# PolusAI/nyxus

Measured on AMD Instinct MI355X. Metric: ROIs/sec (*ALL_GLCM*+*ALL_INTENSITY*, 1024^2 tiles), higher is better.
Workload: dtype f64; 1 GPU; *ALL_GLCM*+*ALL_INTENSITY*, coarse_gray_depth=8, 4 angles, d=1, 1000 synthetic 1024x1024 tiles/GPU x 196 ROIs/tile (disk r=30, 2821 px, bbox 61x61), intensities U[1,4095]; reduce stage on pre-assembled ROI clouds resident in HBM; n_columns=185

## Files before the change

nyxus_amd/csrc/intensity_close.h:

```cpp
#pragma once
#include <hip/hip_runtime.h>
#include "device_math.h"
#include "glcm_rows.h"

namespace nyxhip {

struct RowColumns {
    double* o;
    __device__ __forceinline__ double& operator()(int c) const { return o[c]; }
};

template <class OUT, class SLIDE>
__device__ __forceinline__ void close_sums(const OUT& O, double dn, uint32_t vmin, uint32_t vmax, double tot, double totsq, double mean,
                                           bool have_slide, const SLIDE& slide_range, bool blank)
{
    O(I_MIN) = (double)vmin;
    O(I_MAX) = (double)vmax;
    O(I_RANGE) = (double)vmax - (double)vmin;
    if (have_slide)
        O(I_COVERED_IMAGE_INTENSITY_RANGE) = (double)(vmax - vmin) / slide_range();
    O(I_MEAN) = mean;
    O(I_ENERGY) = totsq;
    O(I_ROOT_MEAN_SQUARED) = sqrt(totsq / dn);
    O(I_INTEGRATED_INTENSITY) = tot;
// ... 50 lines not shown
        const double M2 = acc[1], M3 = acc[2], M4 = acc[3];
        if (M2 != 0.0) {
            const double kurt = n > 4 ? (dn * M4) / (M2 * M2) : 0.0;
            O(I_SKEWNESS) = n > 3 ? (sqrt(dn) * M3) / (M2 * sqrt(M2)) : 0.0;
            O(I_KURTOSIS) = kurt;
            O(I_EXCESS_KURTOSIS) = n > 4 ? kurt - 3 : 0.0;
        }
        const double sd2 = sd * sd, d5 = dn * (sd2 * sd2 * sd), d6 = dn * (sd2 * sd2 * sd2);
        O(I_HYPERSKEWNESS) = d5 == 0. ? 0. : acc[4] / d5;
        O(I_HYPERFLATNESS) = d6 == 0. ? 0. : acc[5] / d6;
    }
}

template <class OUT>
__device__ __forceinline__ void close_robust_mad(const OUT& O, double sadk, uint32_t m2x, uint32_t cle, uint32_t K, double Sx, uint32_t vmin, double dn)
{
    const double dK = (double)K;
    const double sadt = 2.0 * sadk + ((m2x & 1u) ? 2.0 * (double)cle - dn : 0.0);
    O(I_ROBUST_MEAN) = K ? (Sx + dK * (double)vmin) / dK : 0.0;
    O(I_MEDIAN_ABSOLUTE_DEVIATION) = fdiv(sadt * 0.5, dn);
}
template <class OUT>
__device__ __forceinline__ void close_robust_rmad(const OUT& O, double adin, bool fast32, uint32_t K, double Sx, uint32_t lox, uint32_t hix,
                                                  uint32_t n_below, uint32_t n_above)
{
    const double dK = (double)K;
    if (fast32) {
        const double klo = (double)K * (double)lox, khi = (double)K * (double)hix;
        adin -= (double)n_below * fabs(klo - Sx) + (double)n_above * fabs(khi - Sx);
    }
    O(I_ROBUST_MEAN_ABSOLUTE_DEVIATION) = K ? fdiv(fdiv(adin, dK), dK) : 0.0;
}

template <class OUT>
__device__ __forceinline__ void close_quartiles(const OUT& O, double p25, double p75)
{
    O(I_QCOD) = (p75 - p25) / (p75 + p25);
    O(I_INTERQUARTILE_RANGE) = p75 - p25;
}

}
```

nyxus_amd/csrc/roi_features.hip:

```cpp
#include <hip/hip_runtime.h>
#include <type_traits>
#include <algorithm>
#include <cstdlib>
#include <cstdio>
#include "device_math.h"
#include "roi_kernel.h"
#include "launch_util.h"
#include "glcm_rows.h"
#include "glcm_w64.h"
#include "intensity_close.h"
#include "sort_lds.h"
#include "../../include/nyxhip.h"

namespace nyxhip {


enum { S_MEAN = 0, S_P10, S_P90, S_MEDIAN, S_MODE, S_NG };


template <int NW> __device__ __forceinline__ double xw_chain(const double* s_red, int k)
{
    return NW == 1 ? s_red[k] : ((s_red[k] + s_red[8 + k]) + s_red[16 + k]) + s_red[24 + k];
}
template <int NW> __device__ __forceinline__ double xw_pairs(const double* s_red, int k)
{
    return NW == 1 ? s_red[k] : (s_red[k] + s_red[8 + k]) + (s_red[16 + k] + s_red[24 + k]);
}

template <int N, bool GS, int NW = 4>
__device__ __forceinline__ void block_sum(double (&v)[N], double* s_red, int tid)
{
    const int lane = tid & 63, wave = __builtin_amdgcn_readfirstlane(tid >> 6);
    if (N > 4) {
        double t[8];
#pragma unroll
        for (int k = 0; k < 8; k++) t[k] = k < N ? v[k] : 0.0;
        const double tot = wave_transpose_sum8(t, lane);
        if ((lane & 7) == 0 && (lane >> 3) < N)
            s_red[wave * 8 + (lane >> 3)] = tot;
    } else if (N > 2) {
        double t[4];
#pragma unroll
        for (int k = 0; k < 4; k++) t[k] = k < N ? v[k] : 0.0;
        const double tot = wave_transpose_sum4(t);
        if ((lane & 15) == 0 && (lane >> 4) < N)
            s_red[wave * 8 + (lane >> 4)] = tot;
    } else {
#pragma unroll
        for (int k = 0; k < N; k++)
            v[k] = wave_sum(v[k]);
// ... 599 lines not shown
        lds_cu16_t* pc = (lds_cu16_t*)(uintptr_t)(Pd + cj);
        unsigned long long rem = __ballot(act && rc != 0u);
        while (rem) {
            const int r = (int)__builtin_ctzll(rem);
            rem &= rem - 1ull;
            const uint32_t cnt = pc[r * pitch];
            if (cnt >= 7u) { const double p = (double)cnt * inv_sum_p; ent += p * (double)fast_log2f(p + 0.000000001); }
        }
    }
    if constexpr (ROLE == 1) {
        blk_sync<false>();
        blk_sync<false>();
        hxy1c = T2[lane];
        hxy2 = f[lane];
        wav_sync<false>();
    }
    G16_EXIT(5, (uint32_t)(pcol + prow + pxmy + pxpy[0] + pxpy[1] + ent + hxy1c + hxy2) + asm_i + cmax);
    glcm_w64_tail<NG>(Ng, lane, rc, cc, dc, pxpy_c, csum, sum_p, inv_sum_p, pcol, prow, pxmy, pxpy, ent, hxy1c, hxy2, asm_i, cmax, f);
}

#ifdef NYX_STAMP
#define STAMP(i)                                                                          \
    do {                                                                                  \
        unsigned long long t__ = __builtin_readcyclecounter();                            \
        if (tid == 0 && A.stamps) atomicAdd(&A.stamps[i], t__ - t_prev__);                \
        t_prev__ = __builtin_readcyclecounter();                                          \
    } while (0)
#elif defined(NYX_EXIT_AT)
#define STAMP(i) do { if ((i) == NYX_EXIT_AT) return; } while (0)
#else
#define STAMP(i) do { } while (0)
#endif

typedef __attribute__((address_space(3))) uint8_t lds_u8_t;

typedef const __attribute__((address_space(4))) RoiArgs KArgs;
__device__ __forceinline__ KArgs* late_kernarg()
{
    KArgs* p = (KArgs*)__builtin_amdgcn_kernarg_segment_ptr();
    asm volatile("" : "+s"(p));
    return p;
}
template <bool LATE>
struct KView {
    const RoiArgs& a;
    KArgs* p;
    __device__ __forceinline__ explicit KView(const RoiArgs& a_) : a(a_), p(LATE ? late_kernarg() : nullptr) {}
    __device__ __forceinline__ auto operator->() const
    {
        if constexpr (LATE) return p;
        else return &a;
    }
};
template <bool GS, bool C16, bool SPLIT, bool D8, int FAM = 0, int TIER = 4, bool G16 = false, int WIN = 2, int NW = 4, bool DEFER_P = false>
__device__ __forceinline__ void roi_features_body(const RoiArgs& A, const uint64_t slot)
{
    static_assert((NW == 4 && NW == kMaxAngles) || (NW == 8 && G16 && FAM == 4), "one workgroup of four waves per ROI (and a wave per GLCM angle)");
    constexpr int BS = NW * 64;
    extern __shared__ __attribute__((aligned(16))) unsigned char lds_raw[];
    unsigned char* const lds = GS ? A.sp.scratch + (size_t)blockIdx.x * A.sp.stride : lds_raw;
    const int tid = (int)threadIdx.x, lane = tid & 63, wave = __builtin_amdgcn_readfirstlane(tid >> 6);
    uint64_t roi;
    if (!roi_of_slot(A.sp, slot, A.n_roi, roi))
        return;

    auto reg = [&](uint32_t o) -> unsigned char* { return (GS && o < A.L.gs_lds_bytes) ? lds_raw + o : lds + o; };
// ... 23 lines not shown
    const bool do_glcm = FAM == 1 || FAM == 3 || FAM == 4 || (FAM == 0 && (A.mask & NYXHIP_FAM_GLCM) != 0);
    double* const out_row = A.out + roi * A.ld;
#ifdef NYX_STAMP
    unsigned long long t_prev__ = __builtin_readcyclecounter();
#endif

    const uint32_t range = vmax - vmin;
    const bool use_count = C16 ? do_int : (do_int && A.L.count_cap != 0 && range < A.L.count_cap);
    if (C16 && do_int && range >= A.L.count_cap) {
        if (tid == 0) atomicCAS(A.status, 0, NYXHIP_ERR_ROI_TOO_LARGE);
        return;
    }
    uint32_t* s_cnt = (uint32_t*)reg(A.L.cnt);
    uint32_t P2 = 1;
    while (P2 < n)
        P2 <<= 1;
    const bool radix = !C16 && A.L.radix != 0;
    const bool k16 = radix && A.L.radix_k16 != 0;
    if (n == 0 || (do_int && ((use_count || radix) ? n : P2) > A.L.sort_cap) || (do_glcm && area > A.L.dense_cap)) {
        if (SPLIT && A.glcm_ng && tid == 0)
            A.glcm_ng[roi] = 0;
        if (n != 0 && A.sp.defer_large)
            return;
        if (tid == 0 && n != 0)
            atomicCAS(A.status, 0, NYXHIP_ERR_ROI_TOO_LARGE);
        for (int c = tid; c < A.n_cols; c += BS)
            out_row[c] = __longlong_as_double(0x7ff8000000000000LL);
        return;
    }

    const int greyInfo = A.ibsi ? 0 : A.grey_depth;
    if (FAST) __builtin_assume(greyInfo > 0 && greyInfo <= 16);
    if (G16) __builtin_assume(greyInfo > 16 && greyInfo <= 64);
    const double mslope = greyInfo > 0 ? (double)greyInfo / ((double)vmax - 0.) : 0.0;

    for (int c = tid; c < A.n_cols; c += BS)
        out_row[c] = 0.0;
    if (do_glcm) {
        uint32_t* d32 = (uint32_t*)s_dense;
        for (uint32_t i = tid; i < (D8 ? (area + 64 + 3) / 4 : (area + 1) / 2); i += BS)
            d32[i] = 0;
        if (greyInfo < 0)
            for (uint32_t i = tid; i <= A.L.lvl_cap; i += BS)
                s_lvlmap[i] = 0;
    }
    if (do_int) {
        if (use_count) {
            uint4* c4 = (uint4*)s_cnt;
            const uint32_t n16 = C16 ? (range + 8) / 8 : (range + 4) / 4;
            for (uint32_t i = tid; i < n16; i += BS)
                c4[i] = make_uint4(0, 0, 0, 0);
        } else if (!radix) {
            for (uint32_t i = n + tid; i < P2; i += BS)
                s_val[i] = 0xFFFFFFFFu;
        }
    }
    if (tid < 16)
        s_stat[tid] = 0.0;
    grp_sync<GS, NW>();

    STAMP(0);
    unsigned long long sum = 0, sumsq = 0;
    uint32_t lvl_max = 0;
    constexpr int kU = 4;
    const bool small_v = vmax < (1u << 24);
    const __amdgpu_buffer_rsrc_t rs_v = __builtin_amdgcn_make_buffer_rsrc((void*)(A.inten + off), 0, (int)(n * 4u), 0x00020000);
    const __amdgpu_buffer_rsrc_t rs_x = __builtin_amdgcn_make_buffer_rsrc((void*)(A.x + off), 0, (int)(n * 2u), 0x00020000);
    const __amdgpu_buffer_rsrc_t rs_y = __builtin_amdgcn_make_buffer_rsrc((void*)(A.y + off), 0, (int)(n * 2u), 0x00020000);
    auto trip = [&](auto full_c, auto nz_c, auto tiny_c, uint32_t base) {
        constexpr bool FULL = decltype(full_c)::value, NZ = decltype(nz_c)::value, TINY = decltype(tiny_c)::value;
        uint32_t v[kU], px[kU], py[kU];
#pragma unroll
        for (int u = 0; u < kU; u++) {
            const uint32_t i = base + u * BS + tid;
            v[u] = __builtin_amdgcn_raw_buffer_load_b32(rs_v, (int)(i * 4u), 0, 0);
            px[u] = do_glcm ? (uint32_t)(uint16_t)__builtin_amdgcn_raw_buffer_load_b16(rs_x, (int)(i * 2u), 0, 0) : 0u;
            py[u] = do_glcm ? (uint32_t)(uint16_t)__builtin_amdgcn_raw_buffer_load_b16(rs_y, (int)(i * 2u), 0, 0) : 0u;
        }
        uint32_t s32 = 0, q32 = 0;
        const uint32_t i0 = base + tid;
        uint16_t* const val16 = (uint16_t*)s_val + i0;
#pragma unroll
        for (int u = 0; u < kU; u++) {
            if (!FULL && i0 + u * BS >= n)
                continue;
            if (do_int) {
                if (C16) val16[u * BS] = (uint16_t)(v[u] - vmin);
                else if (k16) ((uint16_t*)s_val)[i0 + u * BS] = (uint16_t)(v[u] - vmin);
                else s_val[i0 + u * BS] = v[u];
                const uint32_t sq = (TINY || small_v) ? (uint32_t)__umul24(v[u], v[u]) : (uint32_t)(v[u] * v[u]);
                if (TINY) { s32 += v[u]; q32 += sq; }
                else { sum += v[u]; sumsq += sq; }
// ... 206 lines not shown
        } else {
            for (; base < n; base += kU * BS) trip(F{}, F{}, F{}, base);
        }
    }
    }

    STAMP(1);
    const KView<FAM != 0 || G16> B(A);
    double* const out_row_l = B->out + roi * B->ld;
    if (do_int) {
        double* o = out_row_l + B->col_intensity;
        const double dn = (double)n;
        if ((unsigned long long)n * vmax < (1ull << 32))
            sum = wave_sum_t<uint32_t>((uint32_t)sum);
        else
            sum = wave_sum_u64(sum);
        if (C16) {
            const uint32_t lo24 = wave_sum_t<uint32_t>((uint32_t)sumsq & 0xFFFFFFu), hi = wave_sum_t<uint32_t>((uint32_t)(sumsq >> 24));
            sumsq = ((unsigned long long)hi << 24) + lo24;
        } else
            sumsq = wave_sum_u64(sumsq);
        if (lane == 0) {
            s_red[wave * 8 + 0] = (double)sum;
            s_red[wave * 8 + 1] = (double)sumsq;
        }
        grp_sync<GS, NW>();
        const bool blank = (vmin == 0 && vmax == 0);
#if defined(NYX_NO_FUSED) || defined(NYX_NO_DEFER)
        constexpr bool DEFER = false;
#else
        constexpr bool DEFER = DEFER_P && C16 && !GS;
#endif
        const bool defer = DEFER && !blank;
        double* const rec = DEFER ? B->close_rec + roi * kCloseRec : nullptr;
        if (tid == 0) {
            double tot = 0, totsq = 0;
            for (int wv = 0; wv < NW; wv++) {
                tot += s_red[wv * 8 + 0];
                totsq += s_red[wv * 8 + 1];
            }
            const double mean = tot / dn;
            s_stat[S_MEAN] = mean;
            if (FAST)
                s_stat[S_NG] = bin_pixel(vmin, vmin, vmax, B->glcm_grey_depth) == bin_pixel(vmax, vmin, vmax, B->glcm_grey_depth) ? 1.0 : 0.0;
            if (defer) {
                rec[CR_TOT] = tot;
                rec[CR_TOTSQ] = totsq;
            } else {
                close_sums(RowColumns{o}, dn, vmin, vmax, tot, totsq, mean, B->slide_min && B->slide_max,
                           [&] { return B->slide_max[roi] - B->slide_min[roi]; }, blank);
            }
        }
        grp_sync<GS, NW>();
        const double mean = s_stat[S_MEAN];
        STAMP(2);

        const double binW100 = (double)range / 100.;
        const uint32_t nb = (uint32_t)B->n_hist;
        auto idx100 = [=](uint32_t v) -> int {
            double realIdx = (double)(v - vmin) / binW100;
            return (realIdx != realIdx) ? 0 : (int)realIdx;
        };

        const uint32_t Q = ((range + 1 + NW * 512 - 1) / (NW * 512)) * 512;
        uint32_t* const s_woff = (uint32_t*)(s_stat + 8);
        if (use_count) {
            uint32_t carry = 0, best_c = 0, best_i = 0;
            const uint32_t base = wave * Q;
            if (C16) {
                uint32_t kk[8] = {0, 0, 0, 0, 0, 0, 0, 0};
                uint32_t inv = 0xFFFFu - (base + 8u * (uint32_t)lane);
                uint4* src = (uint4*)((uint16_t*)s_cnt + base + 8u * (uint32_t)lane);
                uint32_t i = base + 8u * (uint32_t)lane;
                for (uint32_t t = 0; t < Q; t += 512, i += 512, inv -= 512, src += 64) {
                    uint4 pk = make_uint4(0, 0, 0, 0);
                    const bool live = i <= range;
                    if (live) pk = *src;
                    kk[0] = max(kk[0], (pk.x << 16) | inv); kk[1] = max(kk[1], (pk.x & 0xFFFF0000u) | inv);
                    kk[2] = max(kk[2], (pk.y << 16) | inv); kk[3] = max(kk[3], (pk.y & 0xFFFF0000u) | inv);
                    kk[4] = max(kk[4], (pk.z << 16) | inv); kk[5] = max(kk[5], (pk.z & 0xFFFF0000u) | inv);
                    kk[6] = max(kk[6], (pk.w << 16) | inv); kk[7] = max(kk[7], (pk.w & 0xFFFF0000u) | inv);
                    const uint32_t A0 = pk.x + (pk.x << 16), A1 = pk.y + (pk.y << 16), A2 = pk.z + (pk.z << 16), A3 = pk.w + (pk.w << 16);
                    const uint32_t T = ((A0 + A1) + (A2 + A3)) >> 16;
                    const uint32_t sc = wave_scan_u32(T);
                    const uint32_t excl = carry + sc - T;
                    const uint32_t o0 = A0 + (excl | (excl << 16));
                    const uint32_t o1 = A1 + __builtin_amdgcn_perm(o0, o0, 0x03020302u);
                    const uint32_t o2 = A2 + __builtin_amdgcn_perm(o1, o1, 0x03020302u);
                    const uint32_t o3 = A3 + __builtin_amdgcn_perm(o2, o2, 0x03020302u);
                    if (live)
// ... 78 lines not shown
        STAMP(3);
        auto SV = [=](uint32_t i) -> uint32_t { return k16 ? vmin + (uint32_t)((const uint16_t*)s_val)[i] : s_val[i]; };
        auto cum = [=](uint32_t i) -> uint32_t {
            const uint32_t wq = (uint32_t)(i >= Q) + (uint32_t)(i >= 2 * Q) + (uint32_t)(i >= 3 * Q);
            return (C16 ? (uint32_t)((const uint16_t*)s_cnt)[i] : s_cnt[i]) + s_woff[wq];
        };

#ifdef NYX_NO_FUSED
        constexpr bool FUSED = false;
#else
        constexpr bool FUSED = C16 && !GS;
#endif
        double acc[6] = {0, 0, 0, 0, 0, 0};
        if (!FUSED || blank) {
            if (!blank) {
                for (uint32_t i = tid; i < n; i += BS) {
                    double d = (double)(C16 ? vmin + ((const uint16_t*)s_val)[i] : SV(i)) - mean;
                    double d2 = d * d;
                    acc[0] += fabs(d);
                    acc[1] += d2;
                    acc[2] += d2 * d;
                    acc[3] += d2 * d2;
                    acc[4] += d2 * d2 * d;
                    acc[5] += d2 * d2 * d2;
                }
                block_sum<6, GS, NW>(acc, s_red, tid);
            }
            if (tid == 0)
                close_central<CovDiv::ieee>(RowColumns{o}, acc, n, dn, mean, blank);
        }
        STAMP(4);

        if (!blank) {
            for (uint32_t t = tid; t < 100 + nb; t += BS) {
                const bool is100 = t < 100;
                const uint32_t b = is100 ? t : t - 100;
                uint32_t lo;
                if (use_count) {
                    auto bin_of = [=](uint32_t dd) -> uint32_t {
                        return is100 ? (uint32_t)idx100(vmin + dd) : to_grayscale(vmin + dd, vmin, range, nb);
                    };
                    uint32_t d;
                    if (range < 65536u) {
                        const double Wl = is100 ? binW100 : (double)range / (double)nb;
                        const double P = (double)b * Wl;
                        const uint32_t m = (uint32_t)(P + 0.5);
                        d = (uint32_t)P + 1;
                        if (b == 0)
                            d = 0;
                        else if (fabs(P - (double)m) < 1e-6)
                            d = bin_of(m) >= b ? m : m + 1;
                    } else {
                        double edge = is100 ? (double)b * binW100 : (double)b * (double)range / (double)nb;
                        d = edge >= (double)range + 1.0 ? range + 1 : (uint32_t)edge;
                        while (d > 0 && bin_of(d - 1) >= b) d--;
                        while (d <= range && bin_of(d) < b) d++;
                    }
                    lo = d > 0 ? cum(d - 1) : 0u;
                } else {
                    uint32_t hi = n;
                    lo = 0;
                    while (lo < hi) {
                        uint32_t mid = (lo + hi) >> 1;
                        uint32_t v = SV(mid);
                        uint32_t idx = is100 ? (uint32_t)idx100(v) : to_grayscale(v, vmin, range, nb);
                        if (idx < b) lo = mid + 1; else hi = mid;
                    }
                }
                if (is100) s_lb100[b] = lo; else s_lbc[b] = lo;
            }
            STAMP(5);
            if (!use_count) {
                uint32_t best_c = 0, best_v = 0;
                for (uint32_t i = tid; i < n; i += BS) {
                    uint32_t v = SV(i);
                    if (i == n - 1 || SV(i + 1) != v) {
                        uint32_t lo = i, hi = i;
                        if (i > 0 && SV(i - 1) == v) {
                            lo = 0;
                            while (lo < hi) {
                                uint32_t mid = (lo + hi) >> 1;
                                if (SV(mid) < v) lo = mid + 1; else hi = mid;
                            }
                        }
                        uint32_t c = i - lo + 1;
                        if (c > best_c || (c == best_c && v < best_v)) { best_c = c; best_v = v; }
                    }
                }
#pragma unroll
                for (int d = 32; d > 0; d >>= 1) {
                    uint32_t oc = __shfl_down(best_c, d, 64), ov = __shfl_down(best_v, d, 64);
                    if (oc > best_c || (oc == best_c && ov < best_v)) { best_c = oc; best_v = ov; }
                }
                if (lane == 0) {
                    s_red[wave * 8 + 0] = (double)best_c;
                    s_red[wave * 8 + 1] = (double)best_v;
                }
                grp_sync<GS, NW>();
                if (tid == 0) {
                    uint32_t mc = 0, mv = 0;
                    for (int wv = 0; wv < NW; wv++) {
                        uint32_t c = (uint32_t)s_red[wv * 8 + 0], v = (uint32_t)s_red[wv * 8 + 1];
                        if (c > mc || (c == mc && v < mv)) { mc = c; mv = v; }
                    }
                    s_stat[S_MODE] = (double)mv;
                }
            }
            grp_sync<GS, NW>();
            STAMP(6);

            if (NW == 1 || wave == 0) {
                const int i0 = lane, i1 = lane + 64;
                const uint32_t r0 = s_lb100[i0], e0 = (i0 < 99 ? s_lb100[i0 + 1] : n);
                const uint32_t r1 = i1 < 100 ? s_lb100[i1] : 0u, e1 = i1 < 100 ? (i1 < 99 ? s_lb100[i1 + 1] : n) : 0u;
                int mywin = -1;
                double mycnt = 0;
#pragma unroll
                for (int q = 0; q < 6; q++) {
                    const double frac = q == 0 ? 0.01 : q == 1 ? 0.1 : q == 2 ? 0.25 : q == 3 ? 0.75 : q == 4 ? 0.9 : 0.99;
                    const double cnt_p = dn * frac;
                    bool m0 = (double)r0 <= cnt_p && cnt_p <= (double)e0;
                    bool m1 = i1 < 100 && (double)r1 <= cnt_p && cnt_p <= (double)e1;
                    unsigned long long b0 = __ballot(m0), b1 = __ballot(m1);
                    int win = b1 ? 64 + (63 - __clzll((long long)b1)) : (b0 ? 63 - __clzll((long long)b0) : -1);
                    if (lane == q) { mywin = win; mycnt = cnt_p; }
                }
                double pv = 0;
                if (mywin >= 0) {
                    uint32_t rs = s_lb100[mywin], bi = (mywin < 99 ? s_lb100[mywin + 1] : n) - rs;
                    pv = (mycnt - (double)rs) * binW100 / (double)bi + (double)vmin + binW100 * (double)mywin;
                }
                double pq[6];
#pragma unroll
                for (int q = 0; q < 6; q++) {
                    pq[q] = readlane_f64(pv, q);
                }
                if (lane == 0) {
                    o[I_P01] = pq[0]; o[I_P10] = pq[1]; o[I_P25] = pq[2]; o[I_P75] = pq[3]; o[I_P90] = pq[4]; o[I_P99] = pq[5];
                    if (!DEFER)
                        close_quartiles(RowColumns{o}, pq[2], pq[3]);
                    s_stat[S_P10] = pq[1];
                    s_stat[S_P90] = pq[4];
                    if (FUSED) {
                        const double p10 = pq[1], p90 = pq[4];
                        uint32_t lox = 0x80000000u, span = 0;
                        if (p10 <= p90 && p90 >= (double)vmin && p10 <= (double)vmax) {
                            const double cl = ceil(p10), fl = floor(p90);
                            const uint32_t lo_v = cl <= (double)vmin ? vmin : (uint32_t)cl, hi_v = fl >= (double)vmax ? vmax : (uint32_t)fl;
                            if (lo_v <= hi_v) { lox = lo_v - vmin; span = hi_v - lo_v; }
                        }
                        const bool empty = span == 0 && lox == 0x80000000u;
                        uint32_t* const s_rob = (uint32_t*)(s_stat + 6);
                        s_rob[0] = lox;
                        s_rob[1] = span;
                        s_rob[2] = (empty || lox == 0) ? 0u : cum(lox - 1);
                        s_rob[3] = empty ? 0u : cum(lox + span);
                    }
                }
            }
            if (NW == 1 || wave == 1) {
                double e = 0, u = 0;
                for (uint32_t k = lane; k < nb; k += 64) {
                    uint32_t ck = (k < nb - 1 ? s_lbc[k + 1] : n) - s_lbc[k];
                    double p = fdiv((double)ck, dn);
                    e += p * log2(p + 2.2e-16);
                    u += p * p;
                }
                e = wave_sum(e);
                u = wave_sum(u);
                if (lane == 0) {
                    o[I_ENTROPY] = -e;
                    o[I_UNIFORMITY] = u;
                }
            }
            if (NW == 1 || wave == 2) {
                uint32_t hi_v, lo_v;
                if (use_count) {
                    auto kth = [&](uint32_t k) -> uint32_t {
                        uint32_t lo = 0, span = range + 1;
                        while (span > 1) {
                            const uint32_t B = (span + 63) >> 6;
                            uint32_t i = lo + mul24((uint32_t)lane + 1, B) - 1;
                            if (i > range) i = range;
                            const unsigned long long hit = __ballot(cum(i) > k);
                            const uint32_t first = hit ? (uint32_t)__builtin_ctzll(hit) : 63u;
                            lo += first * B;
                            span = lo + B > range + 1 ? range + 1 - lo : B;
                        }
                        return lo;
                    };
                    hi_v = vmin + kth(n / 2);
                    lo_v = vmin + kth(n / 2 ? n / 2 - 1 : 0);
                } else {
                    hi_v = SV(n / 2);
                    lo_v = SV(n / 2 ? n / 2 - 1 : 0);
                }
                if (lane == 0) {
                    double median = (n & 1) ? (double)hi_v : (double)(uint32_t)(hi_v + lo_v) / 2.0;
                    o[I_MEDIAN] = median;
                    o[I_MODE] = s_stat[S_MODE];
                    s_stat[S_MEDIAN] = median;
                    if (FUSED) {
                        const uint32_t m2x = (uint32_t)((median - (double)vmin) * 2.0);
                        uint32_t* const s_med = (uint32_t*)(s_stat + 10);
                        s_med[0] = m2x;
                        s_med[1] = (m2x & 1u) ? cum(m2x >> 1) : 0u;
                    }
                }
            }
            grp_sync<GS, NW>();
            STAMP(7);

            const double p10 = s_stat[S_P10], p90 = s_stat[S_P90], median = s_stat[S_MEDIAN];
            if (FUSED) {
                const uint32_t* const s_rob = (const uint32_t*)(s_stat + 6);
                const uint32_t lox = (uint32_t)__builtin_amdgcn_readfirstlane((int)s_rob[0]), span = (uint32_t)__builtin_amdgcn_readfirstlane((int)s_rob[1]);
                const uint32_t hix = lox + span;
                const uint32_t m2x = (uint32_t)__builtin_amdgcn_readfirstlane((int)((const uint32_t*)(s_stat + 10))[0]);
                const uint32_t kmed = m2x >> 1;
                uint32_t sx = 0, sad = 0;
                const double meanx = mean - (double)vmin;
                auto px1 = [&](uint32_t x) {
                    const double d = (double)x - meanx;
                    const double d2 = d * d;
                    acc[0] += fabs(d);
                    acc[1] = __builtin_fma(d, d, acc[1]);
                    acc[2] = __builtin_fma(d2, d, acc[2]);
                    acc[3] = __builtin_fma(d2, d2, acc[3]);
                    const double d4 = d2 * d2;
                    acc[4] = __builtin_fma(d4, d, acc[4]);
                    acc[5] = __builtin_fma(d4, d2, acc[5]);
                    sx += med3_u32_ss(x, lox, hix);
                    asm("v_sad_u32 %0, %1, %2, %0" : "+v"(sad) : "v"(x), "s"(kmed));
                };
                const uint16_t* const pv = (const uint16_t*)s_val + tid;
                const uint32_t n_full = (uint32_t)__builtin_amdgcn_readfirstlane((int)(n / BS)), n_rem = n - n_full * BS;
                {
                    uint32_t k = 0;
                    for (; k + 1 < n_full; k += 2) { px1(pv[k * BS]); px1(pv[(k + 1) * BS]); }
                    if (k < n_full) px1(pv[k * BS]);
// ... 89 lines not shown
            for (uint32_t i = tid; i < n; i += BS) {
                double a = (double)(C16 ? vmin + ((const uint16_t*)s_val)[i] : SV(i));
                if (a >= p10 && a <= p90) {
                    rb[0] += a;
                    rb[1] += 1.0;
                }
                rb[2] += fabs(a - median);
            }
            block_sum<3, GS, NW>(rb, s_red, tid);
            const double mean1090 = rb[1] > 0 ? rb[0] / rb[1] : 0.0;
            double ad[1] = {0};
            for (uint32_t i = tid; i < n; i += BS) {
                double a = (double)(C16 ? vmin + ((const uint16_t*)s_val)[i] : SV(i));
                if (a >= p10 && a <= p90)
                    ad[0] += fabs(a - mean1090);
            }
            block_sum<1, GS, NW>(ad, s_red, tid);
            if (tid == 0) {
                o[I_ROBUST_MEAN] = mean1090;
                o[I_ROBUST_MEAN_ABSOLUTE_DEVIATION] = rb[1] > 0 ? ad[0] / rb[1] : 0.0;
                o[I_MEDIAN_ABSOLUTE_DEVIATION] = fdiv(rb[2], dn);
            }
            }
        }

        STAMP(8);
    }

    STAMP(9);
    if (FAST) {
        double* o = out_row_l + B->col_glcm;
        const int na = B->glcm_na;
        const int Ng = greyInfo, NG1 = Ng + 1, NN = Ng * Ng, cells = NG1 * NG1;
        const bool degenerate = FAM == 3 ? bin_pixel(vmin, vmin, vmax, B->glcm_grey_depth) == bin_pixel(vmax, vmin, vmax, B->glcm_grey_depth) : s_stat[S_NG] != 0.0;
        if (tid == 0)
            B->glcm_ng[roi] = degenerate ? 0u : (uint32_t)Ng;
        if (degenerate) {
            for (int c = tid; c < kGlcmAngled * na + kGlcmAve; c += BS)
                o[c] = B->soft_nan;
            return;
        }
        const bool symmetric = B->glcm_symmetric != 0;
        int slot0 = -1, slot1 = -1, slot2 = -1, slot3 = -1;
#pragma unroll
        for (int q = 0; q < kMaxAngles; q++)
            if (q < na) {
                const int ang = B->glcm_angles[q];
                if (ang == 0) slot0 = q; else if (ang == 45) slot1 = q; else if (ang == 90) slot2 = q; else slot3 = q;
            }
        const bool usual = slot0 >= 0 && slot1 >= 0 && slot2 >= 0 && slot3 >= 0 && !symmetric;
        const bool dpp2 = B->glcm_offset == 1 && w > 64 && w <= 128 && usual;
        const bool dpp = (B->glcm_offset == 1 && w <= 64) || dpp2;
        grp_sync<GS, NW>();
        for (int i = tid; i < na * (dpp ? cells : NN); i += BS)
            s_P[i] = 0;
        grp_sync<GS, NW>();
        STAMP(10);
        if (dpp2) {
            const int rows_per_wave = ((int)h + NW - 1) / NW;
            const int r_begin = wave * rows_per_wave;
            const int r_end = (r_begin + rows_per_wave) < (int)h ? (r_begin + rows_per_wave) : (int)h;
            const uint32_t ng1 = (uint32_t)NG1;
            char* const T0 = (char*)(s_P + slot0 * cells);
            char* const T1 = (char*)(s_P + slot1 * cells);
            char* const T2 = (char*)(s_P + slot2 * cells);
            char* const T3 = (char*)(s_P + slot3 * cells);
            const bool in1 = (uint32_t)lane + 64u < w;
// ... 828 lines not shown
            o[kGlcmAngled * na + j] = na == 4 ? init * 0.25 : na == 2 ? init * 0.5 : na ? init / (double)na : 0.0;
        }
    }
}

constexpr int kCloseBlock = 64;
constexpr uint64_t kCloseCols =
    (1ull << I_MIN) | (1ull << I_MAX) | (1ull << I_RANGE) | (1ull << I_COVERED_IMAGE_INTENSITY_RANGE) | (1ull << I_MEAN) | (1ull << I_ENERGY) |
    (1ull << I_ROOT_MEAN_SQUARED) | (1ull << I_INTEGRATED_INTENSITY) | (1ull << I_UNIFORMITY_PIU) | (1ull << I_MEAN_ABSOLUTE_DEVIATION) |
    (1ull << I_VARIANCE) | (1ull << I_VARIANCE_BIASED) | (1ull << I_STANDARD_DEVIATION) | (1ull << I_STANDARD_DEVIATION_BIASED) | (1ull << I_COV) |
    (1ull << I_STANDARD_ERROR) | (1ull << I_SKEWNESS) | (1ull << I_KURTOSIS) | (1ull << I_EXCESS_KURTOSIS) | (1ull << I_HYPERSKEWNESS) |
    (1ull << I_HYPERFLATNESS) | (1ull << I_ROBUST_MEAN) | (1ull << I_MEDIAN_ABSOLUTE_DEVIATION) | (1ull << I_ROBUST_MEAN_ABSOLUTE_DEVIATION) |
    (1ull << I_QCOD) | (1ull << I_INTERQUARTILE_RANGE);
__global__ __launch_bounds__(kCloseBlock) void intensity_close_kernel(const RoiArgs A)
{
    constexpr int kPitch = __builtin_popcountll(kCloseCols);
#ifndef NYX_CLOSE_DIRECT
    __shared__ double s_o[kCloseBlock * kPitch];
#endif
    const int lane = (int)threadIdx.x;
    uint64_t roi = 0;
    bool mine = roi_of_slot(A.sp, (uint64_t)blockIdx.x * kCloseBlock + (uint64_t)lane, A.n_roi, roi) && glcm_roi_in_launch(A, roi);
    if (mine) mine = A.close_flag[roi] != 0;
    const unsigned long long todo = __ballot(mine);
    if (todo == 0)
        return;
#ifdef NYX_CLOSE_DIRECT
    double* const o = A.out + roi * A.ld + A.col_intensity;
    auto O = [&](int c) -> double& { return o[c]; };
#else
    double* const o = s_o + lane * kPitch;
    auto O = [&](int c) -> double& { return o[__builtin_popcountll(kCloseCols & ((1ull << c) - 1ull))]; };
#endif
    if (mine) {
        A.close_flag[roi] = 0;
        const double* const rec = A.close_rec + roi * kCloseRec;
        const uint32_t* const rw = (const uint32_t*)rec;
        const double* const row = A.out + roi * A.ld + A.col_intensity;
        const uint32_t n = (uint32_t)(A.px_offset[roi + 1] - A.px_offset[roi]);
        const uint32_t vmin = A.min_inten[roi], vmax = A.max_inten[roi];
        const double2 s01 = *(const double2*)(rec + CR_TOT);
        double acc[6];
#pragma unroll
        for (int k = 0; k < 6; k += 2) {
            const double2 t = *(const double2*)(rec + CR_ACC + k);
            acc[k] = t.x; acc[k + 1] = t.y;
        }
        const double sadk = rec[CR_SADK], adin0 = rec[CR_ADIN];
        const bool fast32 = rw[CR_W_FAST32] != 0;
        const uint4 w0 = *(const uint4*)(rw + CR_W_NBELOW), w1 = *(const uint4*)(rw + CR_W_LOX);
        const uint32_t n_below = w0.x, n_above = w0.y, K = w0.z, Sxu = w0.w, lox = w1.x, hix = w1.y, m2x = w1.z, cle = w1.w;
        const double p25 = row[I_P25], p75 = row[I_P75];
#pragma unroll
        for (int c = 0; c < kIntensityCols; c++)
            if ((kCloseCols >> c) & 1ull) O(c) = 0.0;
        const double dn = (double)n;
        constexpr bool blank = false;
        const double tot = s01.x, totsq = s01.y;
        const double mean = tot / dn;
        close_sums(O, dn, vmin, vmax, tot, totsq, mean, A.slide_min && A.slide_max, [&] { return A.slide_max[roi] - A.slide_min[roi]; }, blank);
        close_central<CovDiv::ieee>(O, acc, n, dn, mean, blank);
        const double Sx = (double)Sxu;
        close_robust_mad(O, sadk, m2x, cle, K, Sx, vmin, dn);
        close_robust_rmad(O, adin0, fast32, K, Sx, lox, hix, n_below, n_above);
        close_quartiles(O, p25, p75);
    }
#ifndef NYX_CLOSE_DIRECT
    __syncthreads();
    int mycol = -1;
    {
        int rank = 0;
#pragma unroll
        for (int c = 0; c < kIntensityCols; c++)
            if ((kCloseCols >> c) & 1ull) { if (rank == lane) mycol = c; rank++; }
    }
    double* const dst0 = A.out + A.col_intensity + (mycol >= 0 ? mycol : 0);
#pragma unroll 8
    for (int r = 0; r < kCloseBlock; r++) {
        if (!((todo >> r) & 1ull)) continue;
        const uint64_t rr = readlane_u64(roi, r);
        if (mycol >= 0)
            dst0[rr * A.ld] = s_o[r * kPitch + lane];
    }
#endif
}

size_t glcm_features8_lds(uint32_t ng_cap)
{
    return (2 * glcm8_cnt_bytes(ng_cap) + 8ull * (2 * kMaxAngles * 16 + 2 * kMaxAngles * 32)) * kWaves;
}

size_t glcm_features_lds(uint32_t ng_cap)
{
    const size_t per_wave = (((size_t)4 * kMaxAngles * ng_cap * ng_cap + 15) & ~(size_t)15) + 8ull * (ng_cap + kMaxAngles * 6 * ng_cap + 2 * kMaxAngles * 32);
    return per_wave * kWaves;
}

size_t roi_features_max_lds()
// ... 155 lines not shown
```

nyxus_amd/csrc/roi_kernel.h:

```cpp
#pragma once
#include <stdint.h>
#include <stddef.h>
#include "../../include/nyxhip.h"

namespace nyxhip {

constexpr int kBlock = 256;
constexpr int kWaves = kBlock / 64;
constexpr int kIntensityCols = 36;
constexpr int kGlcmAngled = 30;
constexpr int kGlcmAve = 29;
constexpr int kMaxAngles = 4;

constexpr int kSizeClasses = 5, kClasses = 2 * kSizeClasses;
constexpr uint32_t kClassPx[kSizeClasses - 1] = {256, 4096, 16384, 32768};
constexpr uint32_t kClassSide[kSizeClasses - 1] = {32, 64, 128, 256};
constexpr uint32_t kLdsLevels = 128;
constexpr int kFirstLargeSizeClass = 3;
__host__ __device__ inline int roi_class(uint32_t n, uint32_t w, uint32_t h, uint32_t range, uint32_t lvl = 0)
{
    const uint32_t side = w > h ? w : h;
    int sc = (n <= 256u && side <= 32u) ? 0 : (n <= 4096u && side <= 64u) ? 1 : (n <= 16384u && side <= 128u) ? 2 : (n <= 32768u && side <= 256u) ? 3 : 4;
    if (sc == 2 && range >= 65536u) sc = 3;
    if (sc < 3 && lvl > kLdsLevels) sc = 3;
// ... 39 lines not shown
    uint32_t cnt;
    uint32_t dense;
    uint32_t lvlmap;
    uint32_t P;
    uint32_t gscr;
    uint32_t total;
    uint32_t sort_cap;
    uint32_t count_cap;
    uint32_t cnt16;
    uint32_t dense8;
    uint32_t dense_cap;
    uint32_t ng_cap;
    uint32_t lvl_cap;
    uint32_t app;
    uint32_t g16;
    uint32_t gs_lds_bytes;
    uint32_t radix;
    uint32_t radix_k16;
};

struct WindowSrc {
    const void* inten;
    const void* lab;
    int32_t dt_inten, dt_label;
    uint32_t W, H;
    const uint32_t* tile;
    const uint32_t* label;
    const uint32_t* x0;
    const uint32_t* y0;
    uint32_t xcd_swz;
};
__host__ __device__ inline uint64_t xcd_slot(uint32_t b, uint32_t grid) { const uint32_t per = (grid + 7u) >> 3; return (uint64_t)(b & 7u) * per + (b >> 3); }

constexpr int kCloseRec = 16;
enum {
    CR_TOT = 0, CR_TOTSQ,
    CR_ACC,
    CR_SADK = 9,
    CR_ADIN,
    CR_W_FAST32 = 22,
    CR_W_NBELOW = 24, CR_W_NABOVE, CR_W_K, CR_W_SXU,
    CR_W_LOX, CR_W_HIX, CR_W_M2X, CR_W_CLE
};

struct RoiArgs {
    uint64_t n_roi;
    const uint64_t* px_offset;
    const uint16_t* x;
    const uint16_t* y;
    const uint32_t* inten;
    const uint32_t* bbox_w;
    const uint32_t* bbox_h;
    const uint32_t* min_inten;
    const uint32_t* max_inten;
    const double* slide_min;
    const double* slide_max;
    double* out;
    uint64_t ld;
    int* status;
    unsigned long long* stamps;
    uint32_t mask;
    int32_t n_cols;
    int32_t col_intensity;
    int32_t col_glcm;
    double soft_nan;
    int32_t grey_depth, ibsi, glcm_grey_depth, glcm_offset, glcm_na, glcm_symmetric;
    int32_t glcm_angles[kMaxAngles];
    int32_t n_hist;
    uint32_t* glcm_ws;
    uint32_t* glcm_ng;
    uint32_t glcm_ws_stride;
    uint32_t* census;
    uint32_t small_class;
    uint32_t glcm_feats;
    double* close_rec;
// ... 426 lines not shown
```

nyxus_amd/csrc/device_math.h:

```cpp
#pragma once
#include <hip/hip_runtime.h>
#include <stdint.h>

namespace nyxhip {

__device__ __forceinline__ float fast_log2f(double _x)
{
    float x = (float)_x;
    const float a = -.6296735f;
    const float b = 1.466967f;
    unsigned int ui = __float_as_uint(x);
    int exp_ = (int)((ui & 0x7F800000u) >> 23);
    float signif, fexp;
    if (ui & 0x00400000u) {
        signif = __uint_as_float((ui & 0x007FFFFFu) | 0x3f000000u);
        fexp = (float)exp_ - 126.0f;
    } else {
        signif = __uint_as_float((ui & 0x007FFFFFu) | 0x3f800000u);
        fexp = (float)exp_ - 127.0f;
    }
    signif = signif - 1.0f;
    float t1 = __fmul_rn(__fmul_rn(a, signif), signif);
    float t2 = __fmul_rn(b, signif);
    return __fadd_rn(__fadd_rn(fexp, t1), t2);
// ... 338 lines not shown
    transpose_sum_step<0x141, 4>(v, (lane & 4) != 0);
    transpose_sum_step<0x4E, 2>(v, (lane & 2) != 0);
    transpose_sum_step<0xB1, 1>(v, (lane & 1) != 0);
    return v[0];
}
__device__ __forceinline__ double row16_max(double v)
{
    double o;
    o = dpp_perm<0xB1>(v); v = o > v ? o : v;
    o = dpp_perm<0x4E>(v); v = o > v ? o : v;
    o = dpp_perm<0x141>(v); v = o > v ? o : v;
    o = dpp_perm<0x140>(v); v = o > v ? o : v;
    return v;
}

__device__ __forceinline__ uint32_t lane_plus1(uint32_t v, uint32_t fill)
{
    if (__builtin_constant_p(fill) && fill == 0)
        return (uint32_t)__builtin_amdgcn_update_dpp(0, (int)v, 0x130, 0xF, 0xF, true);
    return (uint32_t)__builtin_amdgcn_update_dpp((int)fill, (int)v, 0x130, 0xF, 0xF, false);
}
__device__ __forceinline__ uint32_t lane_minus1(uint32_t v, uint32_t fill)
{
    if (__builtin_constant_p(fill) && fill == 0)
        return (uint32_t)__builtin_amdgcn_update_dpp(0, (int)v, 0x138, 0xF, 0xF, true);
    return (uint32_t)__builtin_amdgcn_update_dpp((int)fill, (int)v, 0x138, 0xF, 0xF, false);
}


__device__ __forceinline__ uint32_t mul_u24_su(uint32_t a, uint32_t b_uniform)
{
    uint32_t r;
    asm("v_mul_u32_u24 %0, %1, %2" : "=v"(r) : "s"(b_uniform), "v"(a));
    return r;
}

__device__ __forceinline__ int mul_i24(int a, int b)
{
    int r;
    asm("v_mul_i32_i24 %0, %1, %2" : "=v"(r) : "v"(a), "v"(b));
    return r;
}

__device__ __forceinline__ uint32_t med3_u32_ss(uint32_t x, uint32_t lo_uniform, uint32_t hi_uniform)
{
    uint32_t r;
    asm("v_med3_u32 %0, %1, %2, %3" : "=v"(r) : "v"(x), "v"(lo_uniform), "s"(hi_uniform));
    return r;
}

__device__ __forceinline__ uint32_t* cnt16_word(uint32_t* tab, uint32_t ci)
{
    uint32_t t;
    asm("v_and_b32 %0, -2, %1" : "=v"(t) : "v"(ci));
    return (uint32_t*)((char*)tab + (t << 1));
}

__device__ __forceinline__ uint32_t wave_rol1(uint32_t v) { return (uint32_t)__builtin_amdgcn_update_dpp(0, (int)v, 0x134, 0xF, 0xF, true); }
__device__ __forceinline__ uint32_t wave_ror1(uint32_t v) { return (uint32_t)__builtin_amdgcn_update_dpp(0, (int)v, 0x13C, 0xF, 0xF, true); }
__device__ __forceinline__ uint32_t lane_plus1_z(uint32_t v) { return (uint32_t)__builtin_amdgcn_update_dpp(0, (int)v, 0x130, 0xF, 0xF, true); }
__device__ __forceinline__ uint32_t lane_minus1_z(uint32_t v) { return (uint32_t)__builtin_amdgcn_update_dpp(0, (int)v, 0x138, 0xF, 0xF, true); }

template <bool GS>
__device__ __forceinline__ void blk_sync()
{
#ifdef NYX_GS_FULL_FENCE
// ... 36 lines not shown
```

Measured before the change: 100.4 million ROIs/s.

## Defer histogram entropy/uniformity to close kernel and precompute per-ROI slopes once

Moves the histogram entropy and uniformity computation out of the main ROI kernel and into the deferred close kernel. The bin lower bounds are stored as uint16 in an enlarged close record, and the close pass reduces them across lane groups with DPP. The grey-binning slope and bin widths are also computed once per block by spare waves and shared through LDS instead of being recomputed per thread. This trims log2-heavy serial work from the main kernel, but the close record grows from 16 to 20 doubles and the close kernel takes on extra shuffles and scattered global writes.

```diff
diff --git a/nyxus_amd/csrc/intensity_close.h b/nyxus_amd/csrc/intensity_close.h
--- a/nyxus_amd/csrc/intensity_close.h
+++ b/nyxus_amd/csrc/intensity_close.h
@@ -106,6 +106,24 @@
     O(I_ROBUST_MEAN_ABSOLUTE_DEVIATION) = K ? fdiv(fdiv(adin, dK), dK) : 0.0;
 }
 
+__device__ __forceinline__ void hist_bin_terms(uint32_t ck, double dn, double& e, double& u)
+{
+    const double p = fdiv((double)ck, dn);
+    e += p * log2(p + 2.2e-16);
+    u += p * p;
+}
+template <int G>
+__device__ __forceinline__ double hist_group_sum(double v)
+{
+    static_assert(G == 8 || G == 16, "a group is half a DPP row or a whole one");
+    v += dpp_mov0<0x111, 0xF>(v);
+    v += dpp_mov0<0x112, 0xF>(v);
+    v += dpp_mov0<0x114, 0xF>(v);
+    if (G == 16)
+        v += dpp_mov0<0x118, 0xF>(v);
+    return v;
+}
+
 template <class OUT>
 __device__ __forceinline__ void close_quartiles(const OUT& O, double p25, double p75)
 {
diff --git a/nyxus_amd/csrc/roi_features.hip b/nyxus_amd/csrc/roi_features.hip
--- a/nyxus_amd/csrc/roi_features.hip
+++ b/nyxus_amd/csrc/roi_features.hip
@@ -16,6 +16,23 @@
 
 
 enum { S_MEAN = 0, S_P10, S_P90, S_MEDIAN, S_MODE, S_NG };
+enum { S_ONCE0 = 11, S_SLOPE = S_ONCE0, S_BW100, S_BWC };
+
+#if defined(NYX_NO_DEFER_HIST) || defined(NYX_NO_FUSED) || defined(NYX_NO_DEFER)
+constexpr bool kDeferHist = false;
+#else
+constexpr bool kDeferHist = true;
+#endif
+
+template <bool ONCE>
+__device__ __forceinline__ bool glcm_degenerate(uint32_t vmin, uint32_t vmax, int grey_depth, int glcm_grey_depth, const double* s_stat)
+{
+    if (ONCE && glcm_grey_depth == grey_depth && grey_depth > 0) {
+        const double slope = s_stat[S_SLOPE];
+        return bin_matlab(vmin, slope, grey_depth) == bin_matlab(vmax, slope, grey_depth);
+    }
+    return bin_pixel(vmin, vmin, vmax, glcm_grey_depth) == bin_pixel(vmax, vmin, vmax, glcm_grey_depth);
+}
 
 
 template <int NW> __device__ __forceinline__ double xw_chain(const double* s_red, int k)
@@ -770,7 +787,14 @@
     const int greyInfo = A.ibsi ? 0 : A.grey_depth;
     if (FAST) __builtin_assume(greyInfo > 0 && greyInfo <= 16);
     if (G16) __builtin_assume(greyInfo > 16 && greyInfo <= 64);
-    const double mslope = greyInfo > 0 ? (double)greyInfo / ((double)vmax - 0.) : 0.0;
+#ifdef NYX_NO_ONCE
+    constexpr bool ONCE = false;
+#else
+    constexpr bool ONCE = TIER == 8 && (FAM == 1 || FAM == 2 || FAM == 3) && NW == 4 && !GS;
+#endif
+    double mslope = 0.0;
+    if (!ONCE)
+        mslope = greyInfo > 0 ? (double)greyInfo / ((double)vmax - 0.) : 0.0;
 
     for (int c = tid; c < A.n_cols; c += BS)
         out_row[c] = 0.0;
@@ -793,9 +817,23 @@
                 s_val[i] = 0xFFFFFFFFu;
         }
     }
-    if (tid < 16)
+    if (tid < (ONCE ? (int)S_ONCE0 : 16))
         s_stat[tid] = 0.0;
+    if (ONCE) {
+        if (wave == 1 && do_glcm) {
+            const double q = greyInfo > 0 ? (double)greyInfo / ((double)vmax - 0.) : 0.0;
+            if (lane == 0) s_stat[S_SLOPE] = q;
+        } else if (wave == 2 && do_int) {
+            const double q = (double)range / 100.;
+            if (lane == 0) s_stat[S_BW100] = q;
+        } else if (wave == 3 && do_int) {
+            const double q = (double)range / (double)(uint32_t)A.n_hist;
+            if (lane == 0) s_stat[S_BWC] = q;
+        }
+    }
     grp_sync<GS, NW>();
+    if (ONCE && do_glcm)
+        mslope = s_stat[S_SLOPE];
 
     STAMP(0);
     unsigned long long sum = 0, sumsq = 0;
@@ -1068,6 +1106,7 @@
         constexpr bool DEFER = DEFER_P && C16 && !GS;
 #endif
         const bool defer = DEFER && !blank;
+        const bool defer_hist = DEFER && kDeferHist && (uint32_t)B->n_hist <= (uint32_t)kCloseHistBins;
         double* const rec = DEFER ? B->close_rec + roi * kCloseRec : nullptr;
         if (tid == 0) {
             double tot = 0, totsq = 0;
@@ -1078,7 +1117,7 @@
             const double mean = tot / dn;
             s_stat[S_MEAN] = mean;
             if (FAST)
-                s_stat[S_NG] = bin_pixel(vmin, vmin, vmax, B->glcm_grey_depth) == bin_pixel(vmax, vmin, vmax, B->glcm_grey_depth) ? 1.0 : 0.0;
+                s_stat[S_NG] = glcm_degenerate<ONCE>(vmin, vmax, greyInfo, B->glcm_grey_depth, s_stat) ? 1.0 : 0.0;
             if (defer) {
                 rec[CR_TOT] = tot;
                 rec[CR_TOTSQ] = totsq;
@@ -1091,7 +1130,7 @@
         const double mean = s_stat[S_MEAN];
         STAMP(2);
 
-        const double binW100 = (double)range / 100.;
+        const double binW100 = ONCE ? s_stat[S_BW100] : (double)range / 100.;
         const uint32_t nb = (uint32_t)B->n_hist;
         auto idx100 = [=](uint32_t v) -> int {
             double realIdx = (double)(v - vmin) / binW100;
@@ -1246,7 +1285,7 @@
                     };
                     uint32_t d;
                     if (range < 65536u) {
-                        const double Wl = is100 ? binW100 : (double)range / (double)nb;
+                        const double Wl = is100 ? binW100 : ONCE ? s_stat[S_BWC] : (double)range / (double)nb;
                         const double P = (double)b * Wl;
                         const uint32_t m = (uint32_t)(P + 0.5);
                         d = (uint32_t)P + 1;
@@ -1271,7 +1310,9 @@
                         if (idx < b) lo = mid + 1; else hi = mid;
                     }
                 }
-                if (is100) s_lb100[b] = lo; else s_lbc[b] = lo;
+                if (is100) s_lb100[b] = lo;
+                else if (defer_hist) ((uint16_t*)((uint32_t*)rec + CR_W_LB))[b] = (uint16_t)lo;
+                else s_lbc[b] = lo;
             }
             STAMP(5);
             if (!use_count) {
@@ -1362,13 +1403,11 @@
                     }
                 }
             }
-            if (NW == 1 || wave == 1) {
+            if ((NW == 1 || wave == 1) && !defer_hist) {
                 double e = 0, u = 0;
                 for (uint32_t k = lane; k < nb; k += 64) {
                     uint32_t ck = (k < nb - 1 ? s_lbc[k + 1] : n) - s_lbc[k];
-                    double p = fdiv((double)ck, dn);
-                    e += p * log2(p + 2.2e-16);
-                    u += p * p;
+                    hist_bin_terms(ck, dn, e, u);
                 }
                 e = wave_sum(e);
                 u = wave_sum(u);
@@ -1565,7 +1604,7 @@
         double* o = out_row_l + B->col_glcm;
         const int na = B->glcm_na;
         const int Ng = greyInfo, NG1 = Ng + 1, NN = Ng * Ng, cells = NG1 * NG1;
-        const bool degenerate = FAM == 3 ? bin_pixel(vmin, vmin, vmax, B->glcm_grey_depth) == bin_pixel(vmax, vmin, vmax, B->glcm_grey_depth) : s_stat[S_NG] != 0.0;
+        const bool degenerate = FAM == 3 ? glcm_degenerate<ONCE>(vmin, vmax, greyInfo, B->glcm_grey_depth, s_stat) : s_stat[S_NG] != 0.0;
         if (tid == 0)
             B->glcm_ng[roi] = degenerate ? 0u : (uint32_t)Ng;
         if (degenerate) {
@@ -2460,12 +2499,14 @@
     double* const o = s_o + lane * kPitch;
     auto O = [&](int c) -> double& { return o[__builtin_popcountll(kCloseCols & ((1ull << c) - 1ull))]; };
 #endif
+    uint32_t n_mine = 0;
     if (mine) {
         A.close_flag[roi] = 0;
         const double* const rec = A.close_rec + roi * kCloseRec;
         const uint32_t* const rw = (const uint32_t*)rec;
         const double* const row = A.out + roi * A.ld + A.col_intensity;
         const uint32_t n = (uint32_t)(A.px_offset[roi + 1] - A.px_offset[roi]);
+        n_mine = n;
         const uint32_t vmin = A.min_inten[roi], vmax = A.max_inten[roi];
         const double2 s01 = *(const double2*)(rec + CR_TOT);
         double acc[6];
@@ -2492,6 +2533,44 @@
         close_robust_mad(O, sadk, m2x, cle, K, Sx, vmin, dn);
         close_robust_rmad(O, adin0, fast32, K, Sx, lox, hix, n_below, n_above);
         close_quartiles(O, p25, p75);
+    }
+    if (kDeferHist && (uint32_t)A.n_hist <= (uint32_t)kCloseHistBins) {
+        const uint32_t nb = (uint32_t)A.n_hist;
+        auto hist = [&](auto g_c) {
+            constexpr int G = decltype(g_c)::value, R = kCloseBlock / G;
+            const uint32_t k = (uint32_t)lane & (uint32_t)(G - 1);
+            const uint64_t r_any = readlane_u64(roi, (int)__builtin_ctzll(todo));
+            for (int p0 = 0; p0 < G; p0 += 8) {
+                double e[8], u[8];
+                uint64_t r[8];
+#pragma unroll
+                for (int q = 0; q < 8; q++) {
+                    const int src = (p0 + q) * R + lane / G;
+                    r[q] = ((uint64_t)(uint32_t)__shfl((int)(uint32_t)(roi >> 32), src, 64) << 32) | (uint32_t)__shfl((int)(uint32_t)roi, src, 64);
+                    const uint32_t nr = (uint32_t)__shfl((int)n_mine, src, 64);
+                    const bool act = ((todo >> src) & 1ull) != 0 && k < nb;
+                    const uint16_t* const lb = (const uint16_t*)((const uint32_t*)(A.close_rec + (act ? r[q] : r_any) * kCloseRec) + CR_W_LB);
+                    const bool last = !(k < nb - 1);
+                    const uint32_t lo = lb[act ? k : 0u], hi = lb[act && !last ? k + 1 : 0u];
+                    const uint32_t ck = (last ? nr : hi) - lo;
+                    double e1 = 0, u1 = 0;
+                    hist_bin_terms(ck, (double)nr, e1, u1);
+                    e[q] = hist_group_sum<G>(act ? e1 : 0.0);
+                    u[q] = hist_group_sum<G>(act ? u1 : 0.0);
+                }
+#pragma unroll
+                for (int q = 0; q < 8; q++) {
+                    const int src = (p0 + q) * R + lane / G;
+                    if (((todo >> src) & 1ull) != 0 && k == (uint32_t)(G - 1)) {
+                        double* const orow = A.out + r[q] * A.ld + A.col_intensity;
+                        orow[I_ENTROPY] = -e[q];
+                        orow[I_UNIFORMITY] = u[q];
+                    }
+                }
+            }
+        };
+        if (nb <= 8) hist(std::integral_constant<int, 8>{});
+        else hist(std::integral_constant<int, 16>{});
     }
 #ifndef NYX_CLOSE_DIRECT
     __syncthreads();
diff --git a/nyxus_amd/csrc/roi_kernel.h b/nyxus_amd/csrc/roi_kernel.h
--- a/nyxus_amd/csrc/roi_kernel.h
+++ b/nyxus_amd/csrc/roi_kernel.h
@@ -95,7 +95,8 @@
 };
 __host__ __device__ inline uint64_t xcd_slot(uint32_t b, uint32_t grid) { const uint32_t per = (grid + 7u) >> 3; return (uint64_t)(b & 7u) * per + (b >> 3); }
 
-constexpr int kCloseRec = 16;
+constexpr int kCloseRec = 20;
+constexpr int kCloseHistBins = 16;
 enum {
     CR_TOT = 0, CR_TOTSQ,
     CR_ACC,
@@ -103,7 +104,8 @@
     CR_ADIN,
     CR_W_FAST32 = 22,
     CR_W_NBELOW = 24, CR_W_NABOVE, CR_W_K, CR_W_SXU,
-    CR_W_LOX, CR_W_HIX, CR_W_M2X, CR_W_CLE
+    CR_W_LOX, CR_W_HIX, CR_W_M2X, CR_W_CLE,
+    CR_W_LB
 };
 
 struct RoiArgs {
```

Result: no change. 101.0 million ROIs/s, median of 6 (+0.5%).

## Compute percentiles via k-th select instead of building full 100-bin bounds table

Applied to the files above, without the earlier changes.

Drops the block-wide loop that filled all 100 percentile-bin lower bounds plus the coarse bins, and one group barrier. Wave 0 now finds each percentile's and the median's k-th value with an 8-way search, 8 lanes per target, then computes only the two bin bounds each percentile needs. The coarse-bin bounds move into wave 1, which owns the entropy work. This removes work and a sync, but concentrates more serial search in single waves and may shift floating-point edge behaviour of the percentile window choice.

```diff
diff --git a/nyxus_amd/csrc/device_math.h b/nyxus_amd/csrc/device_math.h
--- a/nyxus_amd/csrc/device_math.h
+++ b/nyxus_amd/csrc/device_math.h
@@ -394,6 +394,12 @@
 {
     uint32_t r;
     asm("v_mul_u32_u24 %0, %1, %2" : "=v"(r) : "s"(b_uniform), "v"(a));
+    return r;
+}
+__device__ __forceinline__ uint32_t mad_u24_su(uint32_t a, uint32_t b_uniform, uint32_t c)
+{
+    uint32_t r;
+    asm("v_mad_u32_u24 %0, %1, %2, %3" : "=v"(r) : "s"(b_uniform), "v"(a), "v"(c));
     return r;
 }
 
diff --git a/nyxus_amd/csrc/roi_features.hip b/nyxus_amd/csrc/roi_features.hip
--- a/nyxus_amd/csrc/roi_features.hip
+++ b/nyxus_amd/csrc/roi_features.hip
@@ -681,6 +681,8 @@
 #define STAMP(i) do { } while (0)
 #endif
 
+__constant__ const double kPctFrac[8] = {0.01, 0.1, 0.25, 0.75, 0.9, 0.99, 0.5, 0.5};
+
 typedef __attribute__((address_space(3))) uint8_t lds_u8_t;
 
 typedef const __attribute__((address_space(4))) RoiArgs KArgs;
@@ -1236,9 +1238,8 @@
         STAMP(4);
 
         if (!blank) {
-            for (uint32_t t = tid; t < 100 + nb; t += BS) {
-                const bool is100 = t < 100;
-                const uint32_t b = is100 ? t : t - 100;
+            auto bin_bound = [&](auto is100_t, const uint32_t b) -> uint32_t {
+                constexpr bool is100 = decltype(is100_t)::value;
                 uint32_t lo;
                 if (use_count) {
                     auto bin_of = [=](uint32_t dd) -> uint32_t {
@@ -1271,8 +1272,8 @@
                         if (idx < b) lo = mid + 1; else hi = mid;
                     }
                 }
-                if (is100) s_lb100[b] = lo; else s_lbc[b] = lo;
-            }
+                return lo;
+            };
             STAMP(5);
             if (!use_count) {
                 uint32_t best_c = 0, best_v = 0;
@@ -1310,48 +1311,52 @@
                     s_stat[S_MODE] = (double)mv;
                 }
             }
-            grp_sync<GS, NW>();
             STAMP(6);
 
             if (NW == 1 || wave == 0) {
-                const int i0 = lane, i1 = lane + 64;
-                const uint32_t r0 = s_lb100[i0], e0 = (i0 < 99 ? s_lb100[i0 + 1] : n);
-                const uint32_t r1 = i1 < 100 ? s_lb100[i1] : 0u, e1 = i1 < 100 ? (i1 < 99 ? s_lb100[i1 + 1] : n) : 0u;
-                int mywin = -1;
-                double mycnt = 0;
-#pragma unroll
-                for (int q = 0; q < 6; q++) {
-                    const double frac = q == 0 ? 0.01 : q == 1 ? 0.1 : q == 2 ? 0.25 : q == 3 ? 0.75 : q == 4 ? 0.9 : 0.99;
-                    const double cnt_p = dn * frac;
-                    bool m0 = (double)r0 <= cnt_p && cnt_p <= (double)e0;
-                    bool m1 = i1 < 100 && (double)r1 <= cnt_p && cnt_p <= (double)e1;
-                    unsigned long long b0 = __ballot(m0), b1 = __ballot(m1);
-                    int win = b1 ? 64 + (63 - __clzll((long long)b1)) : (b0 ? 63 - __clzll((long long)b0) : -1);
-                    if (lane == q) { mywin = win; mycnt = cnt_p; }
-                }
-                double pv = 0;
-                if (mywin >= 0) {
-                    uint32_t rs = s_lb100[mywin], bi = (mywin < 99 ? s_lb100[mywin + 1] : n) - rs;
-                    pv = (mycnt - (double)rs) * binW100 / (double)bi + (double)vmin + binW100 * (double)mywin;
-                }
-                double pq[6];
-#pragma unroll
-                for (int q = 0; q < 6; q++) {
-                    pq[q] = readlane_f64(pv, q);
-                }
+                const int g = lane >> 3, sub = lane & 7;
+                const double mycnt = dn * kPctFrac[g];
+                const uint32_t k = g < 6 ? (uint32_t)mycnt : (g == 6 || n / 2 == 0) ? n / 2 : n / 2 - 1;
+                uint32_t xv;
+                if (use_count) {
+                    uint32_t lom1 = 0xFFFFFFFFu, span = range + 1;
+                    while (span > 1) {
+                        const uint32_t B = (span + 7) >> 3;
+                        uint32_t i = mad_u24_su((uint32_t)sub + 1, B, lom1);
+                        if (i > range) i = range;
+                        const unsigned long long hit = __ballot(cum(i) > k);
+                        const uint32_t half = lane < 32 ? (uint32_t)hit : (uint32_t)(hit >> 32);
+                        const uint32_t first = (uint32_t)__builtin_ctz(((half >> (lane & 24)) & 0xFFu) | 0x80u);
+                        lom1 = mad_u24_su(first, B, lom1);
+                        span = B;
+                    }
+                    xv = vmin + lom1 + 1;
+                } else
+                    xv = SV(k);
+                const uint32_t win = min((uint32_t)idx100(xv), 99u);
+                const uint32_t bb = win + (uint32_t)sub;
+                uint32_t bnd = 0;
+                if (g < 6 && sub < 2)
+                    bnd = bb < 100u ? bin_bound(std::true_type{}, bb) : n;
+                const uint32_t rs = bnd, bi = wave_rol1(bnd) - rs;
+                const double pv = (mycnt - (double)rs) * binW100 / (double)bi + (double)vmin + binW100 * (double)win;
+                static_assert(I_P10 == I_P01 + 1 && I_P25 == I_P01 + 2 && I_P75 == I_P01 + 3 && I_P90 == I_P01 + 4 && I_P99 == I_P01 + 5, "P01 .. P99 are adjacent columns");
+                if (g < 6 && sub == 0)
+                    o[I_P01 + g] = pv;
+                const double p10 = readlane_f64(pv, 8), p90 = readlane_f64(pv, 32);
+                const double p25 = DEFER ? 0.0 : readlane_f64(pv, 16), p75 = DEFER ? 0.0 : readlane_f64(pv, 24);
+                const uint32_t hi_v = (uint32_t)__builtin_amdgcn_readlane((int)xv, 48), lo_v = (uint32_t)__builtin_amdgcn_readlane((int)xv, 56);
                 if (lane == 0) {
-                    o[I_P01] = pq[0]; o[I_P10] = pq[1]; o[I_P25] = pq[2]; o[I_P75] = pq[3]; o[I_P90] = pq[4]; o[I_P99] = pq[5];
                     if (!DEFER)
-                        close_quartiles(RowColumns{o}, pq[2], pq[3]);
-                    s_stat[S_P10] = pq[1];
-                    s_stat[S_P90] = pq[4];
+                        close_quartiles(RowColumns{o}, p25, p75);
+                    s_stat[S_P10] = p10;
+                    s_stat[S_P90] = p90;
                     if (FUSED) {
-                        const double p10 = pq[1], p90 = pq[4];
                         uint32_t lox = 0x80000000u, span = 0;
                         if (p10 <= p90 && p90 >= (double)vmin && p10 <= (double)vmax) {
                             const double cl = ceil(p10), fl = floor(p90);
-                            const uint32_t lo_v = cl <= (double)vmin ? vmin : (uint32_t)cl, hi_v = fl >= (double)vmax ? vmax : (uint32_t)fl;
-                            if (lo_v <= hi_v) { lox = lo_v - vmin; span = hi_v - lo_v; }
+                            const uint32_t lo_b = cl <= (double)vmin ? vmin : (uint32_t)cl, hi_b = fl >= (double)vmax ? vmax : (uint32_t)fl;
+                            if (lo_b <= hi_b) { lox = lo_b - vmin; span = hi_b - lo_b; }
                         }
                         const bool empty = span == 0 && lox == 0x80000000u;
                         uint32_t* const s_rob = (uint32_t*)(s_stat + 6);
@@ -1360,46 +1365,6 @@
                         s_rob[2] = (empty || lox == 0) ? 0u : cum(lox - 1);
                         s_rob[3] = empty ? 0u : cum(lox + span);
                     }
-                }
-            }
-            if (NW == 1 || wave == 1) {
-                double e = 0, u = 0;
-                for (uint32_t k = lane; k < nb; k += 64) {
-                    uint32_t ck = (k < nb - 1 ? s_lbc[k + 1] : n) - s_lbc[k];
-                    double p = fdiv((double)ck, dn);
-                    e += p * log2(p + 2.2e-16);
-                    u += p * p;
-                }
-                e = wave_sum(e);
-                u = wave_sum(u);
-                if (lane == 0) {
-                    o[I_ENTROPY] = -e;
-                    o[I_UNIFORMITY] = u;
-                }
-            }
-            if (NW == 1 || wave == 2) {
-                uint32_t hi_v, lo_v;
-                if (use_count) {
-                    auto kth = [&](uint32_t k) -> uint32_t {
-                        uint32_t lo = 0, span = range + 1;
-                        while (span > 1) {
-                            const uint32_t B = (span + 63) >> 6;
-                            uint32_t i = lo + mul24((uint32_t)lane + 1, B) - 1;
-                            if (i > range) i = range;
-                            const unsigned long long hit = __ballot(cum(i) > k);
-                            const uint32_t first = hit ? (uint32_t)__builtin_ctzll(hit) : 63u;
-                            lo += first * B;
-                            span = lo + B > range + 1 ? range + 1 - lo : B;
-                        }
-                        return lo;
-                    };
-                    hi_v = vmin + kth(n / 2);
-                    lo_v = vmin + kth(n / 2 ? n / 2 - 1 : 0);
-                } else {
-                    hi_v = SV(n / 2);
-                    lo_v = SV(n / 2 ? n / 2 - 1 : 0);
-                }
-                if (lane == 0) {
                     double median = (n & 1) ? (double)hi_v : (double)(uint32_t)(hi_v + lo_v) / 2.0;
                     o[I_MEDIAN] = median;
                     o[I_MODE] = s_stat[S_MODE];
@@ -1410,6 +1375,24 @@
                         s_med[0] = m2x;
                         s_med[1] = (m2x & 1u) ? cum(m2x >> 1) : 0u;
                     }
+                }
+            }
+            if (NW == 1 || wave == 1) {
+                for (uint32_t b = lane; b < nb; b += 64)
+                    s_lbc[b] = bin_bound(std::false_type{}, b);
+                wav_sync<GS>();
+                double e = 0, u = 0;
+                for (uint32_t k = lane; k < nb; k += 64) {
+                    uint32_t ck = (k < nb - 1 ? s_lbc[k + 1] : n) - s_lbc[k];
+                    double p = fdiv((double)ck, dn);
+                    e += p * log2(p + 2.2e-16);
+                    u += p * p;
+                }
+                e = wave_sum(e);
+                u = wave_sum(u);
+                if (lane == 0) {
+                    o[I_ENTROPY] = -e;
+                    o[I_UNIFORMITY] = u;
                 }
             }
             grp_sync<GS, NW>();
```

After: 99.89 million ROIs/s before, 101.2 million ROIs/s after (median of 6 runs). 1.01x the previous value.
